# amazon-science/crossnorm-selfnorm

Hardware: AMD Instinct MI355X
Metric: fused CNSN fwd+bwd GB/s vs HBM roofline (higher is better)
Workload: dtype f32

## Files before the change

crossnorm-selfnorm_amd/_ffi.py:

```python
from __future__ import annotations

import ctypes as C
import os

_HERE = os.path.dirname(os.path.abspath(__file__))
LIB_PATH = os.environ.get("CNSN_LIB_PATH") or os.path.join(_HERE, "libcnsn_hip.so")

CNSN_F32, CNSN_BF16, CNSN_F16 = 0, 1, 2
STRATEGY_AUTO, STRATEGY_TWO_PASS, STRATEGY_RESIDENT, STRATEGY_LOCAL, STRATEGY_MONO = 0, 1, 2, 3, 4
ADD_NONE, ADD_PRE, ADD_POST = 0, 1, 2
LAYOUT_NCHW, LAYOUT_NHWC = 0, 1
PATHS = {0: "streaming", 1: "packed", 2: "resident", 3: "local", 4: "mono"}
ABI_VERSION = 9
PERM_INLINE_MAX = 1024
E_UNSUPPORTED = -9


class Problem(C.Structure):
    _fields_ = [
        ("struct_bytes", C.c_int32), ("dtype", C.c_int32),
        ("N", C.c_int32), ("C", C.c_int32), ("H", C.c_int32), ("W", C.c_int32),
        ("cn_active", C.c_int32), ("content_box", C.c_int32 * 4), ("style_box", C.c_int32 * 4),
        ("lam", C.c_float), ("eps_cn", C.c_float),
        ("sn_active", C.c_int32), ("sn_two", C.c_int32), ("sn_training", C.c_int32),
# ... 86 lines not shown
    "cnsn_backward_fused": (C.c_int, [C.POINTER(Problem), C.POINTER(Epilogue), C.c_void_p, C.c_void_p,
                                      C.c_void_p, C.c_void_p, C.POINTER(Gate), C.POINTER(Gate),
                                      C.c_void_p, C.c_void_p, C.c_void_p, C.POINTER(GateGrad),
                                      C.POINTER(GateGrad), C.c_void_p, C.c_size_t, C.c_void_p]),
    "cnsn_which_path": (C.c_int, [C.POINTER(Problem), C.POINTER(Epilogue), C.c_int, C.c_int]),
    "cnsn_keeps_sum": (C.c_int, [C.POINTER(Problem), C.POINTER(Epilogue)]),
    "cnsn_sn_cluster_plan": (C.c_int, [C.POINTER(Problem), C.POINTER(Epilogue), C.c_int]),
    "cnsn_bnrelu_plan": (C.c_int, [C.POINTER(Problem), C.POINTER(Epilogue), C.c_int]),
    "cnsn_bn_block_plan": (C.c_int, [C.POINTER(Problem), C.POINTER(Epilogue)]),
    "cnsn_forward_bn_block": (C.c_int, [C.POINTER(Problem), C.POINTER(Epilogue), C.POINTER(BnTail), C.POINTER(BnTail), C.c_void_p,
                                        C.POINTER(Gate), C.c_void_p, C.c_void_p, C.c_void_p, C.c_void_p, C.c_size_t, C.c_void_p]),
    "cnsn_backward_bn_block": (C.c_int, [C.POINTER(Problem), C.POINTER(Epilogue), C.POINTER(BnTail), C.POINTER(BnTail), C.c_void_p,
                                         C.c_void_p, C.POINTER(Gate), C.c_void_p, C.c_void_p, C.c_void_p, C.c_void_p,
                                         C.POINTER(GateGrad), C.c_void_p, C.c_void_p, C.c_void_p, C.c_void_p, C.c_void_p, C.c_size_t,
                                         C.c_void_p]),
    "cnsn_forward_bnrelu": (C.c_int, [C.POINTER(Problem), C.POINTER(Epilogue), C.POINTER(BnTail), C.c_void_p,
                                      C.POINTER(Gate), C.c_void_p, C.c_void_p, C.c_void_p, C.c_void_p, C.c_void_p,
                                      C.c_size_t, C.c_void_p]),
    "cnsn_backward_bnrelu": (C.c_int, [C.POINTER(Problem), C.POINTER(Epilogue), C.POINTER(BnTail), C.c_void_p, C.c_void_p,
                                       C.c_void_p, C.POINTER(Gate), C.c_void_p, C.c_void_p, C.c_void_p,
                                       C.POINTER(GateGrad), C.c_void_p, C.c_void_p, C.c_void_p, C.c_size_t, C.c_void_p]),
    "cnsn_ibn_plan": (C.c_int, [C.POINTER(Ibn), C.c_int, C.c_int]),
    "cnsn_ibn_saved_floats": (C.c_size_t, [C.POINTER(Ibn)]),
    "cnsn_ibn_workspace_bytes": (C.c_size_t, [C.POINTER(Ibn)]),
    "cnsn_forward_ibn": (C.c_int, [C.POINTER(Ibn), C.c_void_p, C.c_void_p, C.c_void_p, C.c_void_p, C.c_void_p, C.c_size_t,
                                   C.c_void_p]),
    "cnsn_backward_ibn": (C.c_int, [C.POINTER(Ibn), C.c_void_p, C.c_void_p, C.c_void_p, C.c_void_p, C.c_void_p, C.c_void_p,
                                    C.c_void_p, C.c_void_p, C.c_void_p, C.c_void_p, C.c_size_t, C.c_void_p]),
    "cnsn_bn_act_plan": (C.c_int, [C.POINTER(BnAct), C.c_int, C.c_int]),
    "cnsn_bn_act_saved_floats": (C.c_size_t, [C.POINTER(BnAct)]),
# ... 245 lines not shown
```

crossnorm-selfnorm_amd/callers/resnet.py:

```python
import torch
import torch.nn as nn

from .. import functional as _F
from . import _sites
from ._sites import CrossNormSites, make_cnsn, residual_sum
from .bn_act import bn_act
from .ibn import IBN, InstanceNorm2d


class _Bottleneck(nn.Module):
    expansion = 4

    def __init__(self, impl, c_in, planes, stride, downsample, pos, beta, crop, cnsn_type, ibn=None):
        super().__init__()
        c_out = planes * self.expansion
        self.ibn = ibn
        self.conv1 = nn.Conv2d(c_in, planes, 1, bias=False)
        self.bn1 = IBN(planes) if ibn == "a" else nn.BatchNorm2d(planes)
        self.conv2 = nn.Conv2d(planes, planes, 3, stride, 1, bias=False)
        self.bn2 = nn.BatchNorm2d(planes)
        self.conv3 = nn.Conv2d(planes, c_out, 1, bias=False)
        self.bn3 = nn.BatchNorm2d(c_out)
        if ibn == "b":
            self.IN = InstanceNorm2d(c_out, affine=True)
        self.relu = nn.ReLU(inplace=True)
        self.downsample = downsample
        if ibn == "b" and pos == "post":
            cnsn_type = None
        if cnsn_type is not None:
            assert pos in ("residual", "pre", "post", "identity")
            self.cnsn = make_cnsn(impl, cnsn_type, crop, beta, c_in if pos == "pre" else c_out)
        self.pos = pos if cnsn_type is not None else None

    def forward(self, x):
        h = self.cnsn(x) if self.pos == "pre" else x
        h = self.conv1(h)
        h = self.bn1.forward_act(h) if self.ibn == "a" else bn_act(self.bn1, h)
        h = bn_act(self.bn2, self.conv2(h))
        h = self.conv3(h)
        fb = None
        if _sites.FUSE_BLOCK and self.pos in ("post", "residual") and h.is_cuda:
            fb = getattr(getattr(self, "cnsn", None), "forward_bn_block", None)
        if self.ibn == "b":
            skip = x if self.downsample is None else self._skip(x, fb is not None and _F._BN_BLOCK)
            if fb is not None:
                h = fb(h, self.bn3, None, relu=False, add_mode="none")
            else:
                h = self.bn3(h)
                if self.pos == "residual":
                    h = self.cnsn(h)
                elif self.pos == "identity":
                    skip = self.cnsn(skip)
            return self.IN.forward_act(h, skip, relu=True)
        if fb is not None and self.pos == "residual":
            return fb(h, self.bn3, x if self.downsample is None else self._skip(x, _F._BN_BLOCK), relu=True, add_mode="post")
        if fb is not None:
            if self.downsample is None:
                return fb(h, self.bn3, x, relu=True)
            if len(self.downsample) == 2 and isinstance(self.downsample[1], nn.BatchNorm2d):
                return fb(h, self.bn3, self.downsample[0](x), relu=True, identity_bn=self.downsample[1])
            return fb(h, self.bn3, self.downsample(x), relu=True)
        skip = x if self.downsample is None else self.downsample(x)
        if getattr(self, "cnsn", None) is None:
            return bn_act(self.bn3, h, skip)
        return residual_sum(self.cnsn, self.pos, self.bn3(h), skip, relu=True)

    def _skip(self, x, own_launch):
        down = self.downsample
        if own_launch and len(down) == 2 and isinstance(down[1], nn.BatchNorm2d):
            return bn_act(down[1], down[0](x), relu=False)
        return down(x)


class ResNet50CNSN(nn.Module, CrossNormSites):
    def __init__(self, num_classes=1000, layers=(3, 4, 6, 3), active_num=1, pos="post", beta=None, crop=None,
                 cnsn_type="sn", impl=None):
        super().__init__()
        if impl is None:
            from .. import cnsn as impl
        self.conv1 = nn.Conv2d(3, 64, 7, 2, 3, bias=False)
        self.bn1 = nn.BatchNorm2d(64)
        self.relu = nn.ReLU(inplace=True)
        self.maxpool = nn.MaxPool2d(3, 2, 1)
        kw = dict(pos=pos, beta=beta, crop=crop, cnsn_type=cnsn_type)
        c_in = 64
        for i, (planes, blocks) in enumerate(zip((64, 128, 256, 512), layers)):
# ... 3 lines not shown
                down = None
                if b == 0 and (stride != 1 or c_in != planes * 4):
                    down = nn.Sequential(nn.Conv2d(c_in, planes * 4, 1, stride, bias=False), nn.BatchNorm2d(planes * 4))
                units.append(_Bottleneck(impl, c_in, planes, stride if b == 0 else 1, down, **kw))
                c_in = planes * 4
            setattr(self, f"layer{i + 1}", nn.Sequential(*units))
        self.avgpool = nn.AdaptiveAvgPool2d((1, 1))
        self.fc = nn.Linear(c_in, num_classes)
        for m in self.modules():
            if isinstance(m, nn.Conv2d):
                nn.init.kaiming_normal_(m.weight, mode="fan_out", nonlinearity="relu")
            elif isinstance(m, nn.BatchNorm2d):
                nn.init.constant_(m.weight, 1)
                nn.init.constant_(m.bias, 0)
        self._collect_sites(impl, cnsn_type, active_num)

    def forward(self, x, aug=False):
        if aug:
            self._enable_cross_norm()
        x = self.maxpool(bn_act(self.bn1, self.conv1(x)))
        x = self.layer4(self.layer3(self.layer2(self.layer1(x))))
        return self.fc(torch.flatten(self.avgpool(x), 1))
```

crossnorm-selfnorm_amd/callers/resnet_ibn.py:

```python
import torch
import torch.nn as nn

from ._sites import CrossNormSites
from .bn_act import bn_act
from .ibn import InstanceNorm2d
from .resnet import _Bottleneck


class ResNet50IBNCNSN(nn.Module, CrossNormSites):
    def __init__(self, ibn_cfg=("a", "a", "a", None), layers=(3, 4, 6, 3), num_classes=1000, active_num=1, pos="post", beta=None,
                 crop=None, cnsn_type="sn", impl=None):
        super().__init__()
        if impl is None:
            from .. import cnsn as impl
        self.conv1 = nn.Conv2d(3, 64, 7, 2, 3, bias=False)
        self.bn1 = InstanceNorm2d(64, affine=True) if ibn_cfg[0] == "b" else nn.BatchNorm2d(64)
        self.relu = nn.ReLU(inplace=True)
        self.maxpool = nn.MaxPool2d(3, 2, 1)
        kw = dict(pos=pos, beta=beta, crop=crop, cnsn_type=cnsn_type)
        c_in = 64
        for i, (planes, blocks, ibn) in enumerate(zip((64, 128, 256, 512), layers, ibn_cfg)):
            stride = 1 if i == 0 else 2
            units = []
            for b in range(blocks):
# ... 1 lines not shown
                if b == 0 and (stride != 1 or c_in != planes * 4):
                    down = nn.Sequential(nn.Conv2d(c_in, planes * 4, 1, stride, bias=False), nn.BatchNorm2d(planes * 4))
                unit_ibn = None if (ibn == "b" and b < blocks - 1) else ibn
                units.append(_Bottleneck(impl, c_in, planes, stride if b == 0 else 1, down, ibn=unit_ibn, **kw))
                c_in = planes * 4
            setattr(self, f"layer{i + 1}", nn.Sequential(*units))
        self.avgpool = nn.AvgPool2d(7)
        self.fc = nn.Linear(c_in, num_classes)
        for m in self.modules():
            if isinstance(m, nn.Conv2d):
                nn.init.kaiming_normal_(m.weight, mode="fan_out", nonlinearity="relu")
            elif isinstance(m, (nn.BatchNorm2d, nn.InstanceNorm2d, InstanceNorm2d)):
                nn.init.constant_(m.weight, 1)
                nn.init.constant_(m.bias, 0)
        self._collect_sites(impl, cnsn_type, active_num)

    def forward(self, x, aug=False):
        if aug:
            self._enable_cross_norm()
        x = self.conv1(x)
        x = self.bn1.forward_act(x) if isinstance(self.bn1, InstanceNorm2d) else bn_act(self.bn1, x)
        x = self.maxpool(x)
        x = self.layer4(self.layer3(self.layer2(self.layer1(x))))
        return self.fc(torch.flatten(self.avgpool(x), 1))


def resnet50_ibn_a(config, impl=None):
    return ResNet50IBNCNSN(ibn_cfg=("a", "a", "a", None), active_num=config.active_num, pos=config.pos, beta=config.beta,
                           crop=config.crop, cnsn_type=config.cnsn_type, impl=impl)

# ... 5 lines not shown
```

crossnorm-selfnorm_amd/cnsn.py:

```python
from __future__ import annotations

import functools
from dataclasses import dataclass
from typing import Optional, Tuple

import numpy as np
import torch
import torch.nn as nn

from . import functional as _F
from .functional import FusedConfig, GateParams

__all__ = ["calc_ins_mean_std", "instance_norm_mix", "cn_rand_bbox", "cn_op_2ins_space_chan",
           "CrossNorm", "SelfNorm", "CNSN"]

Box = Tuple[int, int, int, int]
_CROPS = ("neither", "style", "content", "both")


def _is_f64(x) -> bool:
    return isinstance(x, torch.Tensor) and x.dtype == torch.float64


def calc_ins_mean_std(x, eps=1e-5):
# ... 244 lines not shown
                x = x + addend
            return torch.relu(x) if relu else x
        kw, g, f, perm, chan = {}, None, None, None, None
        if cn is not None and cn.active:
            if cn_on:
                d = cn._take_draws(x)
                kw.update(cn_active=True, content_box=d.content_box, style_box=d.style_box)
                perm, chan = d.perm, d.chan_perm
            cn.active = False
        if sn is not None:
            skw, g, f = sn._fused_args()
            kw.update(skw)
        cfg = FusedConfig(add_mode=add_mode, relu=bool(relu), **kw)
        return _F.fused_cnsn(x, cfg, perm=perm, chan_perm=chan, g=g, f=f, addend=addend)

    def forward_bn_block(self, conv_out, bn, identity, relu=True, identity_bn=None, add_mode="pre"):
        assert add_mode in ("pre", "post", "none")
        assert (identity is None) == (add_mode == "none")
        cn, sn = self.crossnorm, self.selfnorm
        armed = cn is not None and cn.active

        def plain(m):
            return type(m) is nn.BatchNorm2d and m.affine and m.track_running_stats and m.training
        fused = (plain(bn) and (identity_bn is None or (add_mode == "pre" and plain(identity_bn))) and sn is not None
                 and type(sn) is SelfNorm and sn.f_fc is None and sn._fusable() and not armed and conv_out.is_cuda
                 and (cn is None or type(cn) is CrossNorm)
                 and (identity is None or (identity.shape == conv_out.shape and identity.dtype == conv_out.dtype))
                 and not (add_mode == "none" and relu) and not torch.cuda.is_current_stream_capturing())
        if fused:
            kw, _, _ = sn._fused_args_peek()
            fused = kw["sn_training"] and _F.bn_block_plan(conv_out, FusedConfig(add_mode=add_mode, relu=bool(relu), **kw))
        if not fused:
            skip = identity if identity_bn is None else identity_bn(identity)
            if add_mode == "none":
                y = self(bn(conv_out))
                return torch.relu(y) if relu else y
            return self.forward_block(bn(conv_out), skip, add_mode=add_mode, relu=relu)
        kw, g, _ = sn._fused_args()
        _, bn_eps, bn_mom, bn_counter = SelfNorm._bn_call_state(bn, in_kernel=True)
        cfg = FusedConfig(add_mode=add_mode, relu=bool(relu), **kw)
        extra = ()
        if identity_bn is not None:
            _, e2, m2, c2 = SelfNorm._bn_call_state(identity_bn, in_kernel=True)
            extra = (identity_bn.weight, identity_bn.bias, identity_bn.running_mean, identity_bn.running_var, e2, m2, c2)
        return _F.FusedBnBlock.apply(conv_out, identity, cfg, g.fc_weight, g.bn_weight, g.bn_bias, g.running_mean, g.running_var,
                                     bn.weight, bn.bias, bn.running_mean, bn.running_var, bn_eps, bn_mom, g.num_batches_tracked,
                                     bn_counter, *extra)

    def forward_block_bn(self, x, addend, add_mode, bn, want_y=True):
        assert add_mode in ("none", "pre")
        cn, sn = self.crossnorm, self.selfnorm
        armed = cn is not None and cn.active
        fused = (type(bn) is nn.BatchNorm2d and bn.affine and bn.track_running_stats and sn is not None
                 and type(sn) is SelfNorm and sn.f_fc is None and sn._fusable() and not armed and x.is_cuda
                 and (cn is None or type(cn) is CrossNorm))
        if fused:
            kw, g, _ = sn._fused_args_peek()
            cfg = FusedConfig(add_mode=add_mode, relu=False, **kw)
            fused = _F.bnrelu_plan_cached(x, cfg, torch.is_grad_enabled())
        if not fused:
            y = self.forward_block(x, addend, add_mode=add_mode, relu=False) if add_mode != "none" else self.forward(x)
            return (y if want_y else None), torch.relu(bn(y))
# ... 7 lines not shown
```

crossnorm-selfnorm_amd/csrc/cnsn_fused.hip:

```cpp
#include "../../include/cnsn_hip.h"

#include <hip/hip_runtime.h>

#include "cnsn_fused_stream_kernels.h"
#include "cnsn_host_plan.h"
#include "cnsn_local.h"
#include "cnsn_mono.h"
#include "cnsn_nhwc.h"
#include "cnsn_wide.h"
#include "cnsn_packed.h"
#include "cnsn_resident_fused.h"
#include "cnsn_resident_sn.h"

using namespace cnsn;

namespace {

struct EpiPlan {
    int add;
    int relu;
    const void* addend;
    void* sum_out;
};

// ... 130 lines not shown
    const int st = bn_block_parse(prob, epi, bn, pl, e, false);
    if (st) return st;
    if (bn_skip && e.add != ADD_PRE) return CNSN_E_UNSUPPORTED;
    if (!conv_out || !y || !workspace || !bn_stats || !bn->weight || !bn->bias || !bn->running_mean || !bn->running_var) return CNSN_E_NULL;
    if ((((uintptr_t)conv_out | (uintptr_t)y | (uintptr_t)workspace | (uintptr_t)bn_stats) & 15u) != 0) return CNSN_E_ALIGN;
    if (!gate_ok(g)) return CNSN_E_NULL;
    return nhwc_bnhead_forward(pl, e.add, e.relu, *bn, bn_skip, conv_out, e.addend, gate_dev(g), y, saved, bn_stats, workspace, workspace_bytes,
                               (hipStream_t)stream_);
}

int cnsn_backward_bn_block(const cnsn_problem_t* prob, const cnsn_epilogue_t* epi, const cnsn_bn_tail_t* bn,
                           const cnsn_bn_tail_t* bn_skip, const void* grad_y, const void* conv_out, const cnsn_gate_t* g, const float* saved,
                           const float* bn_stats, void* grad_conv_out, void* grad_identity, const cnsn_gate_grad_t* dg, float* d_bn_weight,
                           float* d_bn_bias, float* d_bn_skip_weight, float* d_bn_skip_bias, void* workspace, size_t workspace_bytes,
                           void* stream_) {
    if (!bn) return CNSN_E_NULL;
    if (bn_skip && (bn_skip->struct_bytes != (int32_t)sizeof(cnsn_bn_tail_t))) return CNSN_E_STRUCT;
    if (bn_skip && (!bn_skip->weight || !d_bn_skip_weight || !d_bn_skip_bias)) return CNSN_E_NULL;
    Plan pl;
    EpiPlan e;
    const int st = bn_block_parse(prob, epi, bn, pl, e, false, false);
    if (st) return st;
    if (bn_skip && e.add != ADD_PRE) return CNSN_E_UNSUPPORTED;
    const bool writes_identity = e.add == ADD_PRE || (e.add == ADD_POST && e.relu);
    if (!grad_y || !conv_out || !grad_conv_out || (writes_identity && !grad_identity) || !saved || !bn_stats || !workspace || !bn->weight)
        return CNSN_E_NULL;
    if ((((uintptr_t)grad_y | (uintptr_t)conv_out | (uintptr_t)grad_conv_out | (uintptr_t)grad_identity | (uintptr_t)workspace |
          (uintptr_t)bn_stats) & 15u) != 0)
        return CNSN_E_ALIGN;
    if (!gate_ok(g) || !dg || !dg->d_fc_weight || !dg->d_bn_weight || !dg->d_bn_bias) return CNSN_E_NULL;
    return nhwc_bnhead_backward(pl, e.add, e.relu, *bn, bn_skip, grad_y, conv_out, e.addend, gate_dev(g), saved, bn_stats, grad_conv_out,
                                grad_identity, gate_grad_dev(dg), d_bn_weight, d_bn_bias, d_bn_skip_weight, d_bn_skip_bias, workspace,
                                workspace_bytes, (hipStream_t)stream_);
}

int cnsn_forward_fused(const cnsn_problem_t* prob, const cnsn_epilogue_t* epi, const void* x, const int64_t* perm,
                       const int64_t* chan_perm, const cnsn_gate_t* g, const cnsn_gate_t* f, void* y, float* saved,
                       void* workspace, size_t workspace_bytes, void* stream_) {
    EpiPlan e;
    int st = parse_epilogue(epi, e);
    if (st) return st;
    if (prob && prob->layout == CNSN_LAYOUT_NHWC) {
        Plan pl;
        st = make_plan(prob, pl);
        if (st) return st;
        if (!x || !y || !workspace) return CNSN_E_NULL;
        if ((((uintptr_t)x | (uintptr_t)y | (uintptr_t)workspace) & 15u) != 0) return CNSN_E_ALIGN;
        if (chan_perm || !nhwc_supported(pl, false)) return CNSN_E_UNSUPPORTED;
// ... 264 lines not shown
```

crossnorm-selfnorm_amd/csrc/cnsn_nhwc.h:

```cpp
#pragma once
#include <type_traits>

#include "cnsn_host_plan.h"

namespace cnsn {

namespace nhwc_host {

inline int vec_of(int dtype) { return 16 / elem_bytes(dtype); }
inline size_t align256(size_t v) { return (v + 255) & ~(size_t)255; }
inline bool aligned16(const void* p) { return ((uintptr_t)p & 15u) == 0; }

template <typename F>
bool dispatch_t(int dtype, F&& f) {
    if (dtype == CNSN_F32) return f(TypeTag<float>{}, IntTag<4>{}), true;
    if (dtype == CNSN_BF16) return f(TypeTag<bf16_t>{}, IntTag<8>{}), true;
    if (dtype == CNSN_F16) return f(TypeTag<_Float16>{}, IntTag<8>{}), true;
    return false;
}

template <typename F>
void with_add(int add, F&& f) {
    if (add == CNSN_ADD_PRE)
        f(IntTag<CNSN_ADD_PRE>{});
// ... 44 lines not shown
int nhwc_fused_forward(Plan& pl, int add, int relu, const void* x, const void* addend, GateDev g, void* y, float* saved,
                       void* workspace, size_t workspace_bytes, hipStream_t stream, void* sum_out = nullptr);
int nhwc_fused_backward(Plan& pl, int add, int relu, const void* gy, const void* x, const void* addend, GateDev g,
                        const float* saved, void* dx, void* d_addend, GateGradDev dg, void* workspace, size_t workspace_bytes,
                        hipStream_t stream);
void nhwc_slim_from_saved(const Plan& pl, const double* saved_d, float* slim, hipStream_t stream);
void nhwc_saved_from_slim(const Plan& pl, const float* slim, int relu, double* saved_d, float* rows, hipStream_t stream);

bool nhwc_bnhead_ok(const Plan& pl, bool check_health = true);
size_t nhwc_bnhead_extra_bytes(const Plan& pl);
int nhwc_bnhead_forward(Plan& pl, int add, int relu, const cnsn_bn_tail_t& bn, const cnsn_bn_tail_t* bn2, const void* conv_out, const void* identity,
                        GateDev gg, void* y, float* saved, float* bn_stats, void* workspace, size_t workspace_bytes, hipStream_t stream);
int nhwc_bnhead_backward(Plan& pl, int add, int relu, const cnsn_bn_tail_t& bn, const cnsn_bn_tail_t* bn2, const void* gy, const void* conv_out,
                         const void* identity, GateDev gg, const float* saved, const float* bn_stats, void* d_conv, void* d_identity,
                         GateGradDev dg, float* dbn_w, float* dbn_b, float* dbn2_w, float* dbn2_b, void* workspace,
                         size_t workspace_bytes, hipStream_t stream);

}
```

crossnorm-selfnorm_amd/csrc/cnsn_nhwc_bnhead_kernels.h:

```cpp
#pragma once
#include "cnsn_nhwc_fused_kernels.h"

#ifndef CNSN_BNHEAD_UA
#define CNSN_BNHEAD_UA 2
#endif
#ifndef CNSN_BNHEAD_WG_PER_CU
#define CNSN_BNHEAD_WG_PER_CU 3
#endif

namespace cnsn {

enum BnSlimRow { SLB_E = SL_ROWS, SLB_DM, SLB_E2, SLB_DM2, SLB_ROWS };
__host__ __device__ inline size_t bn_slim_floats(size_t P, int C) { return (size_t)SLB_ROWS * P + 2 * (size_t)C; }
__host__ __device__ inline double* bn_slim_rstd(float* slim, size_t P) { return reinterpret_cast<double*>(slim + (size_t)SLB_ROWS * P); }
__host__ __device__ inline const double* bn_slim_rstd(const float* slim, size_t P) {
    return reinterpret_cast<const double*>(slim + (size_t)SLB_ROWS * P);
}
enum BnStatRow { BS_MEAN = 0, BS_RSTD, BS_ALPHA, BS_BETA, BS_ROWS };

struct BnHeadDev {
    const float* weight;
    const float* bias;
    float* run_mean;
    float* run_var;
// ... 343 lines not shown
                const size_t e = t.elem(g, t.p0 + t.r + (q - u) * g.rows);
                vc[u] = load_vec_nt<T, VEC>(cv + e);
                if constexpr (RD_B) vb[u] = load_vec_nt<T, VEC>(idt + e);
            }
#pragma unroll
            for (int u = 0; u < U; ++u) emit(vc[u], RD_B ? vb[u] : vc[u], t.elem(g, t.p0 + t.r + (q - u) * g.rows));
        }
        for (; q >= 0; --q) {
            const size_t e = t.elem(g, t.p0 + t.r + q * g.rows);
            const Vec<T, VEC> vc = load_vec_nt<T, VEC>(cv + e);
            emit(vc, RD_B ? load_vec_nt<T, VEC>(idt + e) : vc, e);
        }
    }
}

template <typename T, int VEC, bool KEEP, bool TWO, int ADD = ADD_PRE>
__global__ __launch_bounds__(kBlock, TWO ? 2 : CNSN_BNHEAD_WG_PER_CU) void nhwc_bnhead_bwd_kernel(NhwcBnArgs a, const T* __restrict__ gy,
                                                                                         const T* __restrict__ cv,
                                                                                         const T* __restrict__ idt, T* __restrict__ dconv,
                                                                                         T* __restrict__ didt, GateDev gg, GateGradDev dg) {
    static_assert(!TWO || ADD == ADD_PRE, "a BatchNorm2d on the skip path: the PRE add only");
    constexpr bool RD_B = ADD != ADD_NONE;
    extern __shared__ float lds[];
    __shared__ double red[4 * 2 * kBnGc];
    __shared__ int bar_flag;
    constexpr int GC = kBnGc;
    const NhwcGeom& g = a.f.g;
    const float* __restrict__ row_mu = a.f.slim + (size_t)SL_MU_HI * g.P;
    const float* __restrict__ row_g = a.f.slim + (size_t)SL_G * g.P;
    const float* __restrict__ st_m = a.bn_stats + (size_t)BS_MEAN * g.C;
    const float* __restrict__ st_al = a.bn_stats + (size_t)BS_ALPHA * g.C;
    const float* __restrict__ st_be = a.bn_stats + (size_t)BS_BETA * g.C;
    const float* __restrict__ st2 = a.bn_stats + (size_t)BS_ROWS * g.C;
    const int relu = a.f.relu;

// ... 29 lines not shown
                    } else {
                        nhwc_pair<T, ADD>(to_float(vg.v[j]), bn_out<T>(c, al[j], be[j]), c2, gate[j], 0.f, 0.f, relu, G, X);
                    }
                    acc[0][j] += G;
                    acc[1][j] = fmaf(G, X - mu[j], acc[1][j]);
                    acc[2][j] = fmaf(G, c - mch[j], acc[2][j]);
                    if constexpr (TWO) acc4[0][j] = fmaf(G, c2 - m2ch[j], acc4[0][j]);
                }
            };
            int p = t.p0 + t.r;
            for (; p + g.rows < t.p1; p += 2 * g.rows) {
                Vec<T, VEC> vg[2], vc[2], vb[2];
#pragma unroll
                for (int u = 0; u < 2; ++u) {
                    const size_t e = t.elem(g, p + u * g.rows);
                    vg[u] = nhwc_ld<T, VEC, !KEEP>(gy + e);
                    vc[u] = nhwc_ld<T, VEC, !KEEP>(cv + e);
                    if constexpr (RD_B) vb[u] = nhwc_ld<T, VEC, !KEEP>(idt + e);
                }
#pragma unroll
                for (int u = 0; u < 2; ++u) eat(vg[u], vc[u], RD_B ? vb[u] : vc[u]);
            }
            for (; p < t.p1; p += g.rows) {
                const size_t e = t.elem(g, p);
                const Vec<T, VEC> vc = nhwc_ld<T, VEC, !KEEP>(cv + e);
                eat(nhwc_ld<T, VEC, !KEEP>(gy + e), vc, RD_B ? nhwc_ld<T, VEC, !KEEP>(idt + e) : vc);
            }
        }
        nhwc_rows_sum_part<VEC, 3, kBnBwd>(g, t, acc, 0, lds, a.f.part);
        if constexpr (TWO) nhwc_rows_sum_part<VEC, 1, kBnBwd>(g, t, acc4, 3, lds, a.f.part);
    }
    if (!grid_barrier(a.f.bar, 1, &bar_flag)) {
        nhwc_mark_owed<T, VEC>(g, a.f.ntiles, dconv);
        if constexpr (ADD == ADD_POST) nhwc_mark_owed<T, VEC>(g, a.f.ntiles, didt);
        return;
    }

    for (int slot = blockIdx.x; slot < a.f.ngroups; slot += gridDim.x) {
        const int grp = phase_b_group(slot, a.f.ngroups);
        const int c0 = grp * GC, n = threadIdx.x;
        const bool live = n < g.N;
// ... 164 lines not shown
                }
                const float dX = fmaf(cG[j], G, fmaf(cX[j], X - xr[j], c0[j]));
                if constexpr (TWO)
                    od.v[j] = from_float<T>(fmaf(al2[j], dX, fmaf(e1b[j], c2 - m2ch[j], e0b[j])));
                else
                    od.v[j] = from_float<T>(ADD == ADD_PRE ? dX : G);
                o.v[j] = from_float<T>(fmaf(al[j], dX, fmaf(e1[j], c - mch[j], e0[j])));
            }
            store_vec_nt<T, VEC>(dconv + e, o);
            if constexpr (RD_B) store_vec_nt<T, VEC>(didt + e, od);
        };
        const int cnt = (t.p1 - t.p0 - t.r + g.rows - 1) / g.rows;
        for (int q = cnt - 1; q >= 0; --q) {
            const size_t e = t.elem(g, t.p0 + t.r + q * g.rows);
            const Vec<T, VEC> vc = load_vec_nt<T, VEC>(cv + e);
            emit(load_vec_nt<T, VEC>(gy + e), vc, RD_B ? load_vec_nt<T, VEC>(idt + e) : vc, e);
        }
    }
}

}
```

crossnorm-selfnorm_amd/csrc/cnsn_nhwc_fused.hip:

```cpp
#include "cnsn_nhwc.h"

#include "cnsn_nhwc_fused_host.h"

namespace cnsn {

using namespace nhwc_host;

namespace {
struct FusedWs { float *part, *side; void* bar; size_t bytes; };
FusedWs fused_layout(const NhwcGeom& g, void* workspace) {
    Carver c(workspace);
    return {c.take((size_t)g.S * 2 * g.P * 4), c.take(4 * g.P * 4), c.take<void>(kBarBlock), c.bytes()};
}
struct BnHeadWs { float *part, *side, *chan; void* bar; size_t bytes; };
BnHeadWs bnhead_layout(const NhwcGeom& g, void* workspace) {
    Carver c(workspace);
    return {c.take((size_t)g.S * kBnFwd * g.P * 4), c.take(4 * g.P * 4), c.take(4 * (size_t)g.C * 4), c.take<void>(kBarBlock), c.bytes()};
}
}

NhwcGeom nhwc_fused_geom(const Plan& pl) {
    const cnsn_problem_t& p = pl.pr;
    NhwcGeom g;
    g.N = p.N;
// ... 174 lines not shown
            return a.f.keep ? go(nhwc_bnhead_fwd_kernel<T, VEC, true, true>) : go(nhwc_bnhead_fwd_kernel<T, VEC, false, true>);
        with_add(add, [&](auto at) {
            constexpr int ADD = decltype(at)::value;
            a.f.keep ? go(nhwc_bnhead_fwd_kernel<T, VEC, true, false, ADD>) : go(nhwc_bnhead_fwd_kernel<T, VEC, false, false, ADD>);
        });
    });
    if (knob(K_DEBUG))
        fprintf(stderr, "[cnsn] nhwc bn-block fwd: tiles=%d (S=%d rows=%d tcb=%d) groups=%d keep=%d -> status %d mode=%s\n", a.f.ntiles,
                ng.S, ng.rows, ng.tcb, a.f.ngroups, a.f.keep, status, add_name(add));
    return status;
}

int nhwc_bnhead_backward(Plan& pl, int add, int relu, const cnsn_bn_tail_t& bn, const cnsn_bn_tail_t* bn2, const void* gy,
                         const void* conv_out, const void* identity, GateDev gg, const float* saved, const float* bn_stats, void* d_conv,
                         void* d_identity, GateGradDev dg, float* dbn_w, float* dbn_b, float* dbn2_w, float* dbn2_b, void* workspace,
                         size_t workspace_bytes, hipStream_t stream) {
    if (!nhwc_bnhead_ok(pl, false) || !bn.training || (bn2 && !bn2->training) || !bnhead_mode_ok(add, relu, bn2))
        return CNSN_E_UNSUPPORTED;
    const int eff_add = (add == ADD_POST && !relu) ? ADD_NONE : add;
    if (!saved || !bn_stats || !d_conv || !dbn_w || !dbn_b || (bn2 && (!dbn2_w || !dbn2_b))) return CNSN_E_NULL;
    if (eff_add != ADD_NONE && (!identity || !d_identity)) return CNSN_E_NULL;
    const NhwcGeom ng = nhwc_fused_geom(pl);
    const BnHeadWs w = bnhead_layout(ng, workspace);
    if (workspace_bytes < w.bytes) return CNSN_E_WORKSPACE;
    NhwcBnArgs a = make_bn_args(pl, ng, relu, bn, bn2, const_cast<float*>(bn_stats), w);
    a.f.slim = const_cast<float*>(saved);
    a.dbn_w = dbn_w;
    a.dbn_b = dbn_b;
    a.dbn2_w = dbn2_w;
    a.dbn2_b = dbn2_b;
    a.f.keep = keep_first_read(eff_add != ADD_NONE ? 3 : 2, tensor_bytes(pl));
    int status = CNSN_E_UNSUPPORTED;
    dispatch_t(pl.pr.dtype, [&](auto tt, auto vt) {
        using T = typename decltype(tt)::type;
        constexpr int VEC = decltype(vt)::value;
        const size_t lds = (size_t)3 * ng.rows * ng.tcb * VEC * 4;
        auto go = [&](auto kern) {
            status = launch_fused(pl, kern, lds, a, a.f, w.bar, stream, (const T*)gy, (const T*)conv_out, (const T*)identity,
                                  (T*)d_conv, (T*)d_identity, gg, dg);
        };
        if (bn2)
            return a.f.keep ? go(nhwc_bnhead_bwd_kernel<T, VEC, true, true>) : go(nhwc_bnhead_bwd_kernel<T, VEC, false, true>);
        with_add(eff_add, [&](auto at) {
            constexpr int ADD = decltype(at)::value;
            a.f.keep ? go(nhwc_bnhead_bwd_kernel<T, VEC, true, false, ADD>) : go(nhwc_bnhead_bwd_kernel<T, VEC, false, false, ADD>);
        });
    });
    if (knob(K_DEBUG))
        fprintf(stderr, "[cnsn] nhwc bn-block bwd: tiles=%d (S=%d rows=%d tcb=%d) groups=%d keep=%d -> status %d mode=%s\n", a.f.ntiles,
                ng.S, ng.rows, ng.tcb, a.f.ngroups, a.f.keep, status, add_name(add));
    return status;
}

}
```

crossnorm-selfnorm_amd/functional.py:

```python
from __future__ import annotations

import ctypes as C
import dataclasses
import os
import threading
from dataclasses import dataclass
from typing import Optional, Sequence, Tuple

import torch

from . import _ffi

Box = Tuple[int, int, int, int]

_DTYPES = {torch.float32: _ffi.CNSN_F32, torch.bfloat16: _ffi.CNSN_BF16, torch.float16: _ffi.CNSN_F16}

_strategy = _ffi.STRATEGY_AUTO


def set_strategy(name: str):
    global _strategy
    _strategy = {"auto": _ffi.STRATEGY_AUTO, "two_pass": _ffi.STRATEGY_TWO_PASS,
                 "resident": _ffi.STRATEGY_RESIDENT, "local": _ffi.STRATEGY_LOCAL, "mono": _ffi.STRATEGY_MONO}[name]
    _ffi.forget_plans()
# ... 650 lines not shown
            if torch.cuda.is_current_stream_capturing():
                prob.context, prob.context_bytes = None, 0
            ws = _workspace(ws_bytes, dev)
            epi = _epilogue(cfg, idt)
            st = lib.cnsn_backward_bn_block(C.byref(prob), C.byref(epi), C.byref(hs), C.byref(ss) if ss else None, _ptr(gy), _ptr(x),
                                            C.byref(gate.c), _ptr(saved), _ptr(stats), _ptr(d_conv), _ptr(d_idt) if writes_idt else None,
                                            C.byref(gg),
                                            _ptr(dbw), _ptr(dbb), _ptr(d2w) if skip else None, _ptr(d2b) if skip else None, _ptr(ws),
                                            ws_bytes, _stream(x))
            _ffi.check(st, "cnsn_backward_bn_block")
            outs = _cast_grads(grads, ctx.param_dtypes)
            return (d_conv, d_idt, None, outs[0], outs[1], outs[2], None, None, outs[3], outs[4], None, None, None, None, None, None,
                    outs[5], outs[6], None, None, None, None, None)


def _glue_cfg(cfg: FusedConfig, need_bwd: bool, inline: bool = False):
    cb = cfg.content_box if cfg.content_box is not None else (-1, -1, -1, -1)
    sb = cfg.style_box if cfg.style_box is not None else (-1, -1, -1, -1)
    icfg = [int(cfg.cn_active), *(int(v) for v in cb), *(int(v) for v in sb), int(cfg.sn_active), int(cfg.sn_two),
            int(cfg.sn_training), _strategy, int(need_bwd), _ADD_MODES[cfg.add_mode], int(cfg.relu), int(inline)]
    fcfg = [0.0 if cfg.lam is None else float(cfg.lam), cfg.eps_cn, cfg.eps_sn, cfg.eps_bn, cfg.momentum]
    return icfg, fcfg


_tail_plan_cache = _plan_cache()


def fused_cnsn_tail(x, cfg: FusedConfig, addend, want_y: bool, g: GateParams, bn_w, bn_b, bn_rm, bn_rv, bn_training: bool,
                    bn_eps: float, bn_momentum: float, bn_nbt=None):
    glue = _ffi.glue()
# ... 409 lines not shown
```

include/cnsn_hip.h:

```cpp
#ifndef CNSN_HIP_H_
#define CNSN_HIP_H_

#include <stddef.h>
#include <stdint.h>

#ifdef __cplusplus
extern "C" {
#endif

#define CNSN_ABI_VERSION 9

#define CNSN_PERM_INLINE_MAX 1024

enum cnsn_dtype { CNSN_F32 = 0, CNSN_BF16 = 1, CNSN_F16 = 2, CNSN_F64 = 3 };

enum cnsn_status {
    CNSN_OK = 0,
    CNSN_E_NULL = -1,
    CNSN_E_SHAPE = -2,
    CNSN_E_DTYPE = -3,
    CNSN_E_ALIGN = -4,
    CNSN_E_BOX = -5,
    CNSN_E_WORKSPACE = -6,
    CNSN_E_BATCH = -7,
// ... 138 lines not shown
    CNSN_PATH_LOCAL = 3,
    CNSN_PATH_MONO = 4
};
int cnsn_which_path(const cnsn_problem_t* prob, const cnsn_epilogue_t* epi, int has_chan_perm, int backward);
int cnsn_sn_cluster_plan(const cnsn_problem_t* prob, const cnsn_epilogue_t* epi, int backward);

int cnsn_bn_block_plan(const cnsn_problem_t* prob, const cnsn_epilogue_t* epi);
int cnsn_forward_bn_block(const cnsn_problem_t* prob, const cnsn_epilogue_t* epi, const cnsn_bn_tail_t* bn,
                          const cnsn_bn_tail_t* bn_skip, const void* conv_out, const cnsn_gate_t* g, void* y, float* saved,
                          float* bn_stats, void* workspace, size_t workspace_bytes, void* stream);
int cnsn_backward_bn_block(const cnsn_problem_t* prob, const cnsn_epilogue_t* epi, const cnsn_bn_tail_t* bn,
                           const cnsn_bn_tail_t* bn_skip, const void* grad_y, const void* conv_out, const cnsn_gate_t* g,
                           const float* saved, const float* bn_stats, void* grad_conv_out, void* grad_identity,
                           const cnsn_gate_grad_t* dg, float* d_bn_weight, float* d_bn_bias, float* d_bn_skip_weight,
                           float* d_bn_skip_bias, void* workspace, size_t workspace_bytes, void* stream);

typedef struct cnsn_ibn {
    int32_t struct_bytes;
    int32_t dtype;
    int32_t N, C, H, W;
    int32_t half;
    int32_t relu;
    float eps_in;
    int32_t reserved;
    const float* in_weight;
    const float* in_bias;
    cnsn_bn_tail_t bn;
    void* context;
    uint64_t context_bytes;
} cnsn_ibn_t;
// ... 131 lines not shown
```

Baseline: 8818.

## Fuse fork gradient accumulation into bn-block backward kernel

Each bottleneck block's output now goes out as two aliased outputs, one for the next block's main path and one for its skip path. The backward kernel takes both incoming gradients and sums them on load. This removes the separate autograd add kernel and its extra tensor write/read at every block boundary. The cost is one more input stream per backward kernel, plus more template instantiations and added Python/ABI surface.

```diff
diff --git a/crossnorm-selfnorm_amd/_ffi.py b/crossnorm-selfnorm_amd/_ffi.py
--- a/crossnorm-selfnorm_amd/_ffi.py
+++ b/crossnorm-selfnorm_amd/_ffi.py
@@ -124,6 +124,10 @@
                                          C.c_void_p, C.POINTER(Gate), C.c_void_p, C.c_void_p, C.c_void_p, C.c_void_p,
                                          C.POINTER(GateGrad), C.c_void_p, C.c_void_p, C.c_void_p, C.c_void_p, C.c_void_p, C.c_size_t,
                                          C.c_void_p]),
+    "cnsn_backward_bn_block_fork": (C.c_int, [C.POINTER(Problem), C.POINTER(Epilogue), C.POINTER(BnTail), C.POINTER(BnTail), C.c_void_p,
+                                              C.c_void_p, C.c_void_p, C.POINTER(Gate), C.c_void_p, C.c_void_p, C.c_void_p, C.c_void_p,
+                                              C.POINTER(GateGrad), C.c_void_p, C.c_void_p, C.c_void_p, C.c_void_p, C.c_void_p,
+                                              C.c_size_t, C.c_void_p]),
     "cnsn_forward_bnrelu": (C.c_int, [C.POINTER(Problem), C.POINTER(Epilogue), C.POINTER(BnTail), C.c_void_p,
                                       C.POINTER(Gate), C.c_void_p, C.c_void_p, C.c_void_p, C.c_void_p, C.c_void_p,
                                       C.c_size_t, C.c_void_p]),
diff --git a/crossnorm-selfnorm_amd/callers/resnet.py b/crossnorm-selfnorm_amd/callers/resnet.py
--- a/crossnorm-selfnorm_amd/callers/resnet.py
+++ b/crossnorm-selfnorm_amd/callers/resnet.py
@@ -31,8 +31,11 @@
             assert pos in ("residual", "pre", "post", "identity")
             self.cnsn = make_cnsn(impl, cnsn_type, crop, beta, c_in if pos == "pre" else c_out)
         self.pos = pos if cnsn_type is not None else None
+        self.fork_out = False
 
     def forward(self, x):
+        x, x_skip = x if isinstance(x, tuple) else (x, x)
+        fork = self.fork_out and _F._FORK
         h = self.cnsn(x) if self.pos == "pre" else x
         h = self.conv1(h)
         h = self.bn1.forward_act(h) if self.ibn == "a" else bn_act(self.bn1, h)
@@ -42,7 +45,7 @@
         if _sites.FUSE_BLOCK and self.pos in ("post", "residual") and h.is_cuda:
             fb = getattr(getattr(self, "cnsn", None), "forward_bn_block", None)
         if self.ibn == "b":
-            skip = x if self.downsample is None else self._skip(x, fb is not None and _F._BN_BLOCK)
+            skip = x_skip if self.downsample is None else self._skip(x_skip, fb is not None and _F._BN_BLOCK)
             if fb is not None:
                 h = fb(h, self.bn3, None, relu=False, add_mode="none")
             else:
@@ -53,14 +56,15 @@
                     skip = self.cnsn(skip)
             return self.IN.forward_act(h, skip, relu=True)
         if fb is not None and self.pos == "residual":
-            return fb(h, self.bn3, x if self.downsample is None else self._skip(x, _F._BN_BLOCK), relu=True, add_mode="post")
+            skip = x_skip if self.downsample is None else self._skip(x_skip, _F._BN_BLOCK)
+            return fb(h, self.bn3, skip, relu=True, add_mode="post", fork=fork)
         if fb is not None:
             if self.downsample is None:
-                return fb(h, self.bn3, x, relu=True)
+                return fb(h, self.bn3, x_skip, relu=True, fork=fork)
             if len(self.downsample) == 2 and isinstance(self.downsample[1], nn.BatchNorm2d):
-                return fb(h, self.bn3, self.downsample[0](x), relu=True, identity_bn=self.downsample[1])
-            return fb(h, self.bn3, self.downsample(x), relu=True)
-        skip = x if self.downsample is None else self.downsample(x)
+                return fb(h, self.bn3, self.downsample[0](x_skip), relu=True, identity_bn=self.downsample[1], fork=fork)
+            return fb(h, self.bn3, self.downsample(x_skip), relu=True, fork=fork)
+        skip = x_skip if self.downsample is None else self.downsample(x_skip)
         if getattr(self, "cnsn", None) is None:
             return bn_act(self.bn3, h, skip)
         return residual_sum(self.cnsn, self.pos, self.bn3(h), skip, relu=True)
@@ -70,6 +74,12 @@
         if own_launch and len(down) == 2 and isinstance(down[1], nn.BatchNorm2d):
             return bn_act(down[1], down[0](x), relu=False)
         return down(x)
+
+
+def wire_forks(stages):
+    blocks = [b for stage in stages for b in stage]
+    for b in blocks[:-1]:
+        b.fork_out = True
 
 
 class ResNet50CNSN(nn.Module, CrossNormSites):
@@ -103,6 +113,7 @@
                 nn.init.constant_(m.weight, 1)
                 nn.init.constant_(m.bias, 0)
         self._collect_sites(impl, cnsn_type, active_num)
+        wire_forks((self.layer1, self.layer2, self.layer3, self.layer4))
 
     def forward(self, x, aug=False):
         if aug:
diff --git a/crossnorm-selfnorm_amd/callers/resnet_ibn.py b/crossnorm-selfnorm_amd/callers/resnet_ibn.py
--- a/crossnorm-selfnorm_amd/callers/resnet_ibn.py
+++ b/crossnorm-selfnorm_amd/callers/resnet_ibn.py
@@ -4,7 +4,7 @@
 from ._sites import CrossNormSites
 from .bn_act import bn_act
 from .ibn import InstanceNorm2d
-from .resnet import _Bottleneck
+from .resnet import _Bottleneck, wire_forks
 
 
 class ResNet50IBNCNSN(nn.Module, CrossNormSites):
@@ -39,6 +39,7 @@
                 nn.init.constant_(m.weight, 1)
                 nn.init.constant_(m.bias, 0)
         self._collect_sites(impl, cnsn_type, active_num)
+        wire_forks((self.layer1, self.layer2, self.layer3, self.layer4))
 
     def forward(self, x, aug=False):
         if aug:
diff --git a/crossnorm-selfnorm_amd/cnsn.py b/crossnorm-selfnorm_amd/cnsn.py
--- a/crossnorm-selfnorm_amd/cnsn.py
+++ b/crossnorm-selfnorm_amd/cnsn.py
@@ -282,7 +282,7 @@
         cfg = FusedConfig(add_mode=add_mode, relu=bool(relu), **kw)
         return _F.fused_cnsn(x, cfg, perm=perm, chan_perm=chan, g=g, f=f, addend=addend)
 
-    def forward_bn_block(self, conv_out, bn, identity, relu=True, identity_bn=None, add_mode="pre"):
+    def forward_bn_block(self, conv_out, bn, identity, relu=True, identity_bn=None, add_mode="pre", fork=False):
         assert add_mode in ("pre", "post", "none")
         assert (identity is None) == (add_mode == "none")
         cn, sn = self.crossnorm, self.selfnorm
@@ -302,8 +302,10 @@
             skip = identity if identity_bn is None else identity_bn(identity)
             if add_mode == "none":
                 y = self(bn(conv_out))
-                return torch.relu(y) if relu else y
-            return self.forward_block(bn(conv_out), skip, add_mode=add_mode, relu=relu)
+                y = torch.relu(y) if relu else y
+            else:
+                y = self.forward_block(bn(conv_out), skip, add_mode=add_mode, relu=relu)
+            return (y, y) if fork else y
         kw, g, _ = sn._fused_args()
         _, bn_eps, bn_mom, bn_counter = SelfNorm._bn_call_state(bn, in_kernel=True)
         cfg = FusedConfig(add_mode=add_mode, relu=bool(relu), **kw)
@@ -311,9 +313,10 @@
         if identity_bn is not None:
             _, e2, m2, c2 = SelfNorm._bn_call_state(identity_bn, in_kernel=True)
             extra = (identity_bn.weight, identity_bn.bias, identity_bn.running_mean, identity_bn.running_var, e2, m2, c2)
-        return _F.FusedBnBlock.apply(conv_out, identity, cfg, g.fc_weight, g.bn_weight, g.bn_bias, g.running_mean, g.running_var,
-                                     bn.weight, bn.bias, bn.running_mean, bn.running_var, bn_eps, bn_mom, g.num_batches_tracked,
-                                     bn_counter, *extra)
+        fn = _F.FusedBnBlockFork if fork else _F.FusedBnBlock
+        return fn.apply(conv_out, identity, cfg, g.fc_weight, g.bn_weight, g.bn_bias, g.running_mean, g.running_var,
+                        bn.weight, bn.bias, bn.running_mean, bn.running_var, bn_eps, bn_mom, g.num_batches_tracked,
+                        bn_counter, *extra)
 
     def forward_block_bn(self, x, addend, add_mode, bn, want_y=True):
         assert add_mode in ("none", "pre")
diff --git a/crossnorm-selfnorm_amd/csrc/cnsn_fused.hip b/crossnorm-selfnorm_amd/csrc/cnsn_fused.hip
--- a/crossnorm-selfnorm_amd/csrc/cnsn_fused.hip
+++ b/crossnorm-selfnorm_amd/csrc/cnsn_fused.hip
@@ -168,6 +168,15 @@
                            const float* bn_stats, void* grad_conv_out, void* grad_identity, const cnsn_gate_grad_t* dg, float* d_bn_weight,
                            float* d_bn_bias, float* d_bn_skip_weight, float* d_bn_skip_bias, void* workspace, size_t workspace_bytes,
                            void* stream_) {
+    return cnsn_backward_bn_block_fork(prob, epi, bn, bn_skip, grad_y, nullptr, conv_out, g, saved, bn_stats, grad_conv_out, grad_identity,
+                                       dg, d_bn_weight, d_bn_bias, d_bn_skip_weight, d_bn_skip_bias, workspace, workspace_bytes, stream_);
+}
+
+int cnsn_backward_bn_block_fork(const cnsn_problem_t* prob, const cnsn_epilogue_t* epi, const cnsn_bn_tail_t* bn,
+                                const cnsn_bn_tail_t* bn_skip, const void* grad_y, const void* grad_y2, const void* conv_out,
+                                const cnsn_gate_t* g, const float* saved, const float* bn_stats, void* grad_conv_out, void* grad_identity,
+                                const cnsn_gate_grad_t* dg, float* d_bn_weight, float* d_bn_bias, float* d_bn_skip_weight,
+                                float* d_bn_skip_bias, void* workspace, size_t workspace_bytes, void* stream_) {
     if (!bn) return CNSN_E_NULL;
     if (bn_skip && (bn_skip->struct_bytes != (int32_t)sizeof(cnsn_bn_tail_t))) return CNSN_E_STRUCT;
     if (bn_skip && (!bn_skip->weight || !d_bn_skip_weight || !d_bn_skip_bias)) return CNSN_E_NULL;
@@ -179,13 +188,13 @@
     const bool writes_identity = e.add == ADD_PRE || (e.add == ADD_POST && e.relu);
     if (!grad_y || !conv_out || !grad_conv_out || (writes_identity && !grad_identity) || !saved || !bn_stats || !workspace || !bn->weight)
         return CNSN_E_NULL;
-    if ((((uintptr_t)grad_y | (uintptr_t)conv_out | (uintptr_t)grad_conv_out | (uintptr_t)grad_identity | (uintptr_t)workspace |
-          (uintptr_t)bn_stats) & 15u) != 0)
+    if ((((uintptr_t)grad_y | (uintptr_t)grad_y2 | (uintptr_t)conv_out | (uintptr_t)grad_conv_out | (uintptr_t)grad_identity |
+          (uintptr_t)workspace | (uintptr_t)bn_stats) & 15u) != 0)
         return CNSN_E_ALIGN;
     if (!gate_ok(g) || !dg || !dg->d_fc_weight || !dg->d_bn_weight || !dg->d_bn_bias) return CNSN_E_NULL;
     return nhwc_bnhead_backward(pl, e.add, e.relu, *bn, bn_skip, grad_y, conv_out, e.addend, gate_dev(g), saved, bn_stats, grad_conv_out,
                                 grad_identity, gate_grad_dev(dg), d_bn_weight, d_bn_bias, d_bn_skip_weight, d_bn_skip_bias, workspace,
-                                workspace_bytes, (hipStream_t)stream_);
+                                workspace_bytes, (hipStream_t)stream_, grad_y2);
 }
 
 int cnsn_forward_fused(const cnsn_problem_t* prob, const cnsn_epilogue_t* epi, const void* x, const int64_t* perm,
diff --git a/crossnorm-selfnorm_amd/csrc/cnsn_nhwc.h b/crossnorm-selfnorm_amd/csrc/cnsn_nhwc.h
--- a/crossnorm-selfnorm_amd/csrc/cnsn_nhwc.h
+++ b/crossnorm-selfnorm_amd/csrc/cnsn_nhwc.h
@@ -82,6 +82,6 @@
 int nhwc_bnhead_backward(Plan& pl, int add, int relu, const cnsn_bn_tail_t& bn, const cnsn_bn_tail_t* bn2, const void* gy, const void* conv_out,
                          const void* identity, GateDev gg, const float* saved, const float* bn_stats, void* d_conv, void* d_identity,
                          GateGradDev dg, float* dbn_w, float* dbn_b, float* dbn2_w, float* dbn2_b, void* workspace,
-                         size_t workspace_bytes, hipStream_t stream);
+                         size_t workspace_bytes, hipStream_t stream, const void* gy2 = nullptr);
 
 }
diff --git a/crossnorm-selfnorm_amd/csrc/cnsn_nhwc_bnhead_kernels.h b/crossnorm-selfnorm_amd/csrc/cnsn_nhwc_bnhead_kernels.h
--- a/crossnorm-selfnorm_amd/csrc/cnsn_nhwc_bnhead_kernels.h
+++ b/crossnorm-selfnorm_amd/csrc/cnsn_nhwc_bnhead_kernels.h
@@ -381,11 +381,23 @@
     }
 }
 
-template <typename T, int VEC, bool KEEP, bool TWO, int ADD = ADD_PRE>
+template <typename T, int VEC, bool NT, bool FORK>
+__device__ __forceinline__ Vec<T, VEC> bn_ld_grad(const T* __restrict__ gy, const T* __restrict__ gy2, size_t e) {
+    Vec<T, VEC> g = nhwc_ld<T, VEC, NT>(gy + e);
+    if constexpr (FORK) {
+        const Vec<T, VEC> h = nhwc_ld<T, VEC, NT>(gy2 + e);
+#pragma unroll
+        for (int j = 0; j < VEC; ++j) g.v[j] = from_float<T>(to_float(g.v[j]) + to_float(h.v[j]));
+    }
+    return g;
+}
+
+template <typename T, int VEC, bool KEEP, bool TWO, int ADD = ADD_PRE, bool FORK = false>
 __global__ __launch_bounds__(kBlock, TWO ? 2 : CNSN_BNHEAD_WG_PER_CU) void nhwc_bnhead_bwd_kernel(NhwcBnArgs a, const T* __restrict__ gy,
                                                                                          const T* __restrict__ cv,
                                                                                          const T* __restrict__ idt, T* __restrict__ dconv,
-                                                                                         T* __restrict__ didt, GateDev gg, GateGradDev dg) {
+                                                                                         T* __restrict__ didt, GateDev gg, GateGradDev dg,
+                                                                                         const T* __restrict__ gy2) {
     static_assert(!TWO || ADD == ADD_PRE, "a BatchNorm2d on the skip path: the PRE add only");
     constexpr bool RD_B = ADD != ADD_NONE;
     extern __shared__ float lds[];
@@ -445,7 +457,7 @@
 #pragma unroll
                 for (int u = 0; u < 2; ++u) {
                     const size_t e = t.elem(g, p + u * g.rows);
-                    vg[u] = nhwc_ld<T, VEC, !KEEP>(gy + e);
+                    vg[u] = bn_ld_grad<T, VEC, !KEEP, FORK>(gy, gy2, e);
                     vc[u] = nhwc_ld<T, VEC, !KEEP>(cv + e);
                     if constexpr (RD_B) vb[u] = nhwc_ld<T, VEC, !KEEP>(idt + e);
                 }
@@ -455,7 +467,7 @@
             for (; p < t.p1; p += g.rows) {
                 const size_t e = t.elem(g, p);
                 const Vec<T, VEC> vc = nhwc_ld<T, VEC, !KEEP>(cv + e);
-                eat(nhwc_ld<T, VEC, !KEEP>(gy + e), vc, RD_B ? nhwc_ld<T, VEC, !KEEP>(idt + e) : vc);
+                eat(bn_ld_grad<T, VEC, !KEEP, FORK>(gy, gy2, e), vc, RD_B ? nhwc_ld<T, VEC, !KEEP>(idt + e) : vc);
             }
         }
         nhwc_rows_sum_part<VEC, 3, kBnBwd>(g, t, acc, 0, lds, a.f.part);
@@ -650,9 +662,9 @@
         for (int q = cnt - 1; q >= 0; --q) {
             const size_t e = t.elem(g, t.p0 + t.r + q * g.rows);
             const Vec<T, VEC> vc = load_vec_nt<T, VEC>(cv + e);
-            emit(load_vec_nt<T, VEC>(gy + e), vc, RD_B ? load_vec_nt<T, VEC>(idt + e) : vc, e);
-        }
-    }
-}
-
-}
+            emit(bn_ld_grad<T, VEC, true, FORK>(gy, gy2, e), vc, RD_B ? load_vec_nt<T, VEC>(idt + e) : vc, e);
+        }
+    }
+}
+
+}
diff --git a/crossnorm-selfnorm_amd/csrc/cnsn_nhwc_fused.hip b/crossnorm-selfnorm_amd/csrc/cnsn_nhwc_fused.hip
--- a/crossnorm-selfnorm_amd/csrc/cnsn_nhwc_fused.hip
+++ b/crossnorm-selfnorm_amd/csrc/cnsn_nhwc_fused.hip
@@ -212,10 +212,11 @@
 int nhwc_bnhead_backward(Plan& pl, int add, int relu, const cnsn_bn_tail_t& bn, const cnsn_bn_tail_t* bn2, const void* gy,
                          const void* conv_out, const void* identity, GateDev gg, const float* saved, const float* bn_stats, void* d_conv,
                          void* d_identity, GateGradDev dg, float* dbn_w, float* dbn_b, float* dbn2_w, float* dbn2_b, void* workspace,
-                         size_t workspace_bytes, hipStream_t stream) {
+                         size_t workspace_bytes, hipStream_t stream, const void* gy2) {
     if (!nhwc_bnhead_ok(pl, false) || !bn.training || (bn2 && !bn2->training) || !bnhead_mode_ok(add, relu, bn2))
         return CNSN_E_UNSUPPORTED;
     const int eff_add = (add == ADD_POST && !relu) ? ADD_NONE : add;
+    if (gy2 && add == ADD_POST && !relu) return CNSN_E_UNSUPPORTED;
     if (!saved || !bn_stats || !d_conv || !dbn_w || !dbn_b || (bn2 && (!dbn2_w || !dbn2_b))) return CNSN_E_NULL;
     if (eff_add != ADD_NONE && (!identity || !d_identity)) return CNSN_E_NULL;
     const NhwcGeom ng = nhwc_fused_geom(pl);
@@ -227,7 +228,7 @@
     a.dbn_b = dbn_b;
     a.dbn2_w = dbn2_w;
     a.dbn2_b = dbn2_b;
-    a.f.keep = keep_first_read(eff_add != ADD_NONE ? 3 : 2, tensor_bytes(pl));
+    a.f.keep = keep_first_read((eff_add != ADD_NONE ? 3 : 2) + (gy2 ? 1 : 0), tensor_bytes(pl));
     int status = CNSN_E_UNSUPPORTED;
     dispatch_t(pl.pr.dtype, [&](auto tt, auto vt) {
         using T = typename decltype(tt)::type;
@@ -235,19 +236,26 @@
         const size_t lds = (size_t)3 * ng.rows * ng.tcb * VEC * 4;
         auto go = [&](auto kern) {
             status = launch_fused(pl, kern, lds, a, a.f, w.bar, stream, (const T*)gy, (const T*)conv_out, (const T*)identity,
-                                  (T*)d_conv, (T*)d_identity, gg, dg);
-        };
-        if (bn2)
-            return a.f.keep ? go(nhwc_bnhead_bwd_kernel<T, VEC, true, true>) : go(nhwc_bnhead_bwd_kernel<T, VEC, false, true>);
-        with_add(eff_add, [&](auto at) {
-            constexpr int ADD = decltype(at)::value;
-            a.f.keep ? go(nhwc_bnhead_bwd_kernel<T, VEC, true, false, ADD>) : go(nhwc_bnhead_bwd_kernel<T, VEC, false, false, ADD>);
-        });
-    });
-    if (knob(K_DEBUG))
-        fprintf(stderr, "[cnsn] nhwc bn-block bwd: tiles=%d (S=%d rows=%d tcb=%d) groups=%d keep=%d -> status %d mode=%s\n", a.f.ntiles,
-                ng.S, ng.rows, ng.tcb, a.f.ngroups, a.f.keep, status, add_name(add));
-    return status;
-}
-
-}
+                                  (T*)d_conv, (T*)d_identity, gg, dg, (const T*)gy2);
+        };
+        with_flag(gy2 != nullptr, [&](auto ft) {
+            constexpr bool FORK = decltype(ft)::value;
+            if (bn2) {
+                a.f.keep ? go(nhwc_bnhead_bwd_kernel<T, VEC, true, true, ADD_PRE, FORK>)
+                         : go(nhwc_bnhead_bwd_kernel<T, VEC, false, true, ADD_PRE, FORK>);
+                return;
+            }
+            with_add(eff_add, [&](auto at) {
+                constexpr int ADD = decltype(at)::value;
+                a.f.keep ? go(nhwc_bnhead_bwd_kernel<T, VEC, true, false, ADD, FORK>)
+                         : go(nhwc_bnhead_bwd_kernel<T, VEC, false, false, ADD, FORK>);
+            });
+        });
+    });
+    if (knob(K_DEBUG))
+        fprintf(stderr, "[cnsn] nhwc bn-block bwd: tiles=%d (S=%d rows=%d tcb=%d) groups=%d keep=%d -> status %d mode=%s%s\n", a.f.ntiles,
+                ng.S, ng.rows, ng.tcb, a.f.ngroups, a.f.keep, status, add_name(add), gy2 ? " fork" : "");
+    return status;
+}
+
+}
diff --git a/crossnorm-selfnorm_amd/functional.py b/crossnorm-selfnorm_amd/functional.py
--- a/crossnorm-selfnorm_amd/functional.py
+++ b/crossnorm-selfnorm_amd/functional.py
@@ -688,6 +688,57 @@
                     outs[5], outs[6], None, None, None, None, None)
 
 
+_FORK = os.environ.get("CNSN_FORK", "1") != "0"
+
+
+def _fork_forward(ctx, *args):
+    y = FusedBnBlock.forward(ctx, *args)
+    ctx.set_materialize_grads(False)
+    return y, y.detach()
+
+
+def _fork_backward(ctx, g_a, g_b):
+    if g_a is None or g_b is None:
+        g = g_a if g_b is None else g_b
+        return FusedBnBlock.backward(ctx, g) if g is not None else (None,) * 23
+    x, idt, saved, stats = ctx.saved_tensors
+    cfg = ctx.cfg
+
+    def as_it_is(g):
+        return g.dtype == x.dtype and g.is_contiguous(memory_format=torch.channels_last) and g.data_ptr() % 16 == 0
+    if (cfg.add_mode == "post" and not cfg.relu) or not (as_it_is(g_a) and as_it_is(g_b)):
+        return FusedBnBlock.backward(ctx, torch.add(g_a, g_b))
+    with torch.cuda.device(x.device):
+        lib = _ffi.lib()
+        prob, gate, skip = ctx.prob, ctx.gate, ctx.skip
+        dev = x.device
+        hs = ctx.head.struct()
+        ss = skip.struct() if skip else None
+        writes_idt = cfg.add_mode != "none"
+        d_conv = _out_like(x)
+        d_idt = _out_like(x) if writes_idt else None
+        grads, gg = _gate_grad_views(x.shape[1], dev, 4)
+        dbw, dbb, d2w, d2b = grads[3:]
+        ws_bytes = _sizes(prob)[1]
+        _context(prob, dev)
+        if torch.cuda.is_current_stream_capturing():
+            prob.context, prob.context_bytes = None, 0
+        ws = _workspace(ws_bytes, dev)
+        epi = _epilogue(cfg, idt)
+        st = lib.cnsn_backward_bn_block_fork(C.byref(prob), C.byref(epi), C.byref(hs), C.byref(ss) if ss else None, _ptr(g_a), _ptr(g_b),
+                                             _ptr(x), C.byref(gate.c), _ptr(saved), _ptr(stats), _ptr(d_conv), _ptr(d_idt), C.byref(gg),
+                                             _ptr(dbw), _ptr(dbb), _ptr(d2w) if skip else None, _ptr(d2b) if skip else None, _ptr(ws),
+                                             ws_bytes, _stream(x))
+        _ffi.check(st, "cnsn_backward_bn_block_fork")
+        outs = _cast_grads(grads, ctx.param_dtypes)
+        return (d_conv, d_idt, None, outs[0], outs[1], outs[2], None, None, outs[3], outs[4], None, None, None, None, None, None,
+                outs[5], outs[6], None, None, None, None, None)
+
+
+FusedBnBlockFork = type(torch.autograd.Function)(
+    "FusedBnBlock", (torch.autograd.Function,), {"forward": staticmethod(_fork_forward), "backward": staticmethod(_fork_backward)})
+
+
 def _glue_cfg(cfg: FusedConfig, need_bwd: bool, inline: bool = False):
     cb = cfg.content_box if cfg.content_box is not None else (-1, -1, -1, -1)
     sb = cfg.style_box if cfg.style_box is not None else (-1, -1, -1, -1)
diff --git a/include/cnsn_hip.h b/include/cnsn_hip.h
--- a/include/cnsn_hip.h
+++ b/include/cnsn_hip.h
@@ -176,6 +176,11 @@
                            const float* saved, const float* bn_stats, void* grad_conv_out, void* grad_identity,
                            const cnsn_gate_grad_t* dg, float* d_bn_weight, float* d_bn_bias, float* d_bn_skip_weight,
                            float* d_bn_skip_bias, void* workspace, size_t workspace_bytes, void* stream);
+int cnsn_backward_bn_block_fork(const cnsn_problem_t* prob, const cnsn_epilogue_t* epi, const cnsn_bn_tail_t* bn,
+                                const cnsn_bn_tail_t* bn_skip, const void* grad_y, const void* grad_y2, const void* conv_out,
+                                const cnsn_gate_t* g, const float* saved, const float* bn_stats, void* grad_conv_out,
+                                void* grad_identity, const cnsn_gate_grad_t* dg, float* d_bn_weight, float* d_bn_bias,
+                                float* d_bn_skip_weight, float* d_bn_skip_bias, void* workspace, size_t workspace_bytes, void* stream);
 
 typedef struct cnsn_ibn {
     int32_t struct_bytes;
```

Result: faster. 8911 (median of 6 runs) (+1.1%).
